# aditya-v-kallappa/FInCFlow

Hardware: AMD Instinct MI355X
Metric: inverse images/sec (+ fwd+logdet ms/img in `forward`), 3x3 conv @64x64x96 (higher is better)
Workload: dtype f32

## Files before the change

fincflow_amd/_lib.py:

```python
import ctypes
import os

HERE = os.path.dirname(os.path.abspath(__file__))
LIB_OVERRIDE = os.environ.get("FINCFLOW_LIB") or None
LIB_PATH = LIB_OVERRIDE or os.path.join(HERE, "libfinc_hip.so")

OK = 0
ALGO = {"auto": 0, "strict": 1, "mfma": 2}

SYMBOLS = [
    "finc_version", "finc_status_string", "finc_last_hip_error", "finc_canonicalize_weights_f32",
    "finc_check_invariant_f32", "finc_workspace_bytes", "finc_inverse_algo_for", "finc_forward_algo_for",
    "finc_inverse_f32", "finc_forward_f32", "finc_pack_inverse_weights_f32", "finc_pack_forward_weights_f32",
    "finc_inverse_packed_f32", "finc_forward_packed_f32", "finc_backward_f32", "finc_backward_workspace_bytes",
    "finc_inverse_workspace_bytes", "finc_pack_inverse_weights_affine_f32",
    "finc_canonicalize_weights_f64", "finc_inverse_f64", "finc_forward_f64",
    "finc_f64_workspace_bytes", "finc_inverse_f64_algo", "finc_forward_f64_algo",
    "finc_inverse_kernel_variant", "finc_debug_attr_table_insert", "finc_debug_inverse_table_row",
    "finc_mix_supported_f32", "finc_mix_f32", "finc_pack_forward_weights_affine_f32", "finc_debug_hlp_timeouts",
    "finc_build_flags", "finc_inverse_packed_premultiplied_f32", "finc_inverse_premultiplied_supported", "finc_clear_fault", "finc_debug_backward_variant", "finc_debug_set_forward_form",
    "finc_debug_row_chunks", "finc_debug_inverse_remainder_images",
    "finc_inverse_affine_supported", "finc_fault_pending", "finc_runtime_switches",
    "finc_debug_clock_probe_begin", "finc_debug_clock_probe_end",
    "finc_mix_backward_workspace_bytes", "finc_mix_backward_f32",
    "finc_coupling_supported_f32", "finc_coupling_workspace_bytes", "finc_coupling_f32", "finc_coupling_backward_f32",
    "finc_bias_relu_f32",
    "finc_actnorm_workspace_bytes", "finc_actnorm_f32", "finc_actnorm_backward_f32", "finc_actnorm_init_f32",
    "finc_adjoint_weights_f32", "finc_lead_product_f32", "finc_negate_f32", "finc_inverse_backward_workspace_bytes",
    "finc_inverse_backward_f32",
    "finc_coupling_reverse_backward_f32", "finc_actnorm_reverse_backward_f32",
    "finc_coupling_reverse_logdet_f32", "finc_coupling_reverse_logdet_backward_f32",
]

ABI_VERSION = 104
ACTNORM_ABI_VERSION = 105
INVERSE_BACKWARD_ABI_VERSION = 107
REVERSE_BACKWARD_ABI_VERSION = 108
SAMPLE_LOGDET_ABI_VERSION = 109

_lib = None


class FincError(RuntimeError):
    pass


def lib():
    global _lib
    if _lib is not None:
        return _lib
    if not os.path.exists(LIB_PATH):
        raise FincError(
            f"{LIB_PATH} not found: build it with `python -c 'import __graft_entry__ as g; g.build()'` "
            "(or `make -C fincflow_amd/csrc`).  fincflow_amd has no CPU / PyTorch fallback.")
    L = ctypes.CDLL(LIB_PATH)
    vp, i, u, sz = ctypes.c_void_p, ctypes.c_int, ctypes.c_uint, ctypes.c_size_t
    try:
        L.finc_version.restype = i
        have = int(L.finc_version())
    except AttributeError:
        raise FincError(f"{LIB_PATH} does not export finc_version: not a build of libfinc_hip.so") from None
    if have < ABI_VERSION:
        raise FincError(f"{LIB_PATH} reports finc_version() = {have}, this package needs at least {ABI_VERSION}: rebuild it "
                        "(`make -C fincflow_amd/csrc`)" + (" or unset FINCFLOW_LIB" if LIB_OVERRIDE else ""))
    if have < ACTNORM_ABI_VERSION:
        raise FincError(f"{LIB_PATH} reports finc_version() = {have}, the ActNorm entry points (finc_actnorm_f32, "
                        f"finc_actnorm_backward_f32, finc_actnorm_init_f32) came with {ACTNORM_ABI_VERSION}: rebuild it "
                        "(`make -C fincflow_amd/csrc`)" + (" or unset FINCFLOW_LIB" if LIB_OVERRIDE else ""))
    if have < INVERSE_BACKWARD_ABI_VERSION:
        raise FincError(f"{LIB_PATH} reports finc_version() = {have}, the backward through the inverse (finc_adjoint_weights_f32, "
                        f"finc_inverse_backward_f32) came with {INVERSE_BACKWARD_ABI_VERSION}: rebuild it "
                        "(`make -C fincflow_amd/csrc`)" + (" or unset FINCFLOW_LIB" if LIB_OVERRIDE else ""))
    if have < REVERSE_BACKWARD_ABI_VERSION:
        raise FincError(f"{LIB_PATH} reports finc_version() = {have}, the backwards of the reverse direction "
                        f"(finc_coupling_reverse_backward_f32, finc_actnorm_reverse_backward_f32) came with "
                        f"{REVERSE_BACKWARD_ABI_VERSION}: rebuild it "
                        "(`make -C fincflow_amd/csrc`)" + (" or unset FINCFLOW_LIB" if LIB_OVERRIDE else ""))
    if have < SAMPLE_LOGDET_ABI_VERSION:
        raise FincError(f"{LIB_PATH} reports finc_version() = {have}, the coupling's reverse with its log-det "
                        f"(finc_coupling_reverse_logdet_f32, finc_coupling_reverse_logdet_backward_f32) came with "
                        f"{SAMPLE_LOGDET_ABI_VERSION}: rebuild it "
                        "(`make -C fincflow_amd/csrc`)" + (" or unset FINCFLOW_LIB" if LIB_OVERRIDE else ""))
    L.finc_build_flags.restype = u
    L.finc_clear_fault.restype = i
    L.finc_status_string.restype = ctypes.c_char_p
    L.finc_status_string.argtypes = [i]
    L.finc_last_hip_error.restype = ctypes.c_char_p
    L.finc_canonicalize_weights_f32.argtypes = [vp, vp, i, i, i, i, u, vp]
    L.finc_check_invariant_f32.argtypes = [vp, i, i, i, i, vp]
    L.finc_workspace_bytes.restype = sz
    L.finc_workspace_bytes.argtypes = [i, i, i, i]
    L.finc_inverse_algo_for.argtypes = [i, i, i, i, i]
    L.finc_forward_algo_for.argtypes = [i, i, i, i, i]
    run = [vp, vp, vp, i, i, i, i, i, i, i, u, i, vp, sz, vp]
    L.finc_inverse_f32.argtypes = run
    L.finc_forward_f32.argtypes = run
    L.finc_pack_inverse_weights_f32.argtypes = [vp, vp, i, i, i, i, vp]
    L.finc_pack_inverse_weights_affine_f32.argtypes = [vp, vp, vp, vp, i, i, i, i, vp]
    L.finc_pack_forward_weights_f32.argtypes = [vp, vp, i, i, i, i, vp]
    L.finc_pack_forward_weights_affine_f32.argtypes = [vp, vp, vp, vp, i, i, i, i, vp]
    runp = [vp, vp, vp, i, i, i, i, i, i, i, u, vp]
    L.finc_inverse_packed_f32.argtypes = runp
    L.finc_inverse_packed_premultiplied_f32.argtypes = runp
    L.finc_inverse_premultiplied_supported.argtypes = [i, i, i, i, i, i, i]
    L.finc_inverse_affine_supported.argtypes = [i, i, i, i, i, i, i]
    L.finc_fault_pending.restype = i
    L.finc_runtime_switches.argtypes = [ctypes.c_char_p, sz]
    L.finc_debug_clock_probe_begin.argtypes = [i, i]
    L.finc_debug_clock_probe_end.argtypes = [ctypes.POINTER(ctypes.c_double)]
    L.finc_forward_packed_f32.argtypes = runp
    L.finc_backward_workspace_bytes.restype = sz
    L.finc_inverse_workspace_bytes.restype = sz
    L.finc_inverse_workspace_bytes.argtypes = [i, i, i, i, i, i, i]
    L.finc_backward_workspace_bytes.argtypes = [i, i, i, i, i, i, i]
# ... 10 lines not shown
    L.finc_debug_attr_table_insert.argtypes = [i, sz]
    L.finc_debug_inverse_table_row.argtypes = [i, ctypes.POINTER(ctypes.c_int)]
    L.finc_debug_hlp_timeouts.argtypes = [ctypes.POINTER(ctypes.c_uint)]
    L.finc_debug_backward_variant.argtypes = [i, i, i, i, i, i, i, ctypes.POINTER(ctypes.c_int)]
    L.finc_debug_inverse_remainder_images.argtypes = [i, i, i, i, i, i, i]
    L.finc_debug_row_chunks.argtypes = [ctypes.c_longlong, ctypes.c_longlong, i, i, i, i]
    L.finc_debug_set_forward_form.argtypes = [i]
    L.finc_mix_supported_f32.argtypes = [i]
    L.finc_mix_f32.argtypes = [vp, vp, vp, vp, i, i, i, vp]
    L.finc_mix_backward_workspace_bytes.restype = sz
    L.finc_mix_backward_workspace_bytes.argtypes = [i, i, i]
    L.finc_mix_backward_f32.argtypes = [vp, vp, vp, vp, vp, vp, i, i, i, vp, sz, vp]
    L.finc_coupling_supported_f32.argtypes = [i]
    L.finc_coupling_workspace_bytes.restype = sz
    L.finc_coupling_workspace_bytes.argtypes = [i, i, i]
    L.finc_coupling_f32.argtypes = [vp, vp, vp, vp, vp, vp, i, i, i, i, vp, sz, vp]
    L.finc_coupling_backward_f32.argtypes = [vp, vp, vp, vp, vp, vp, vp, vp, vp, vp, i, i, i, vp, sz, vp]
    L.finc_bias_relu_f32.argtypes = [vp, vp, vp, i, i, i, vp]
    L.finc_actnorm_workspace_bytes.restype = sz
    L.finc_actnorm_workspace_bytes.argtypes = [i, i, i]
    L.finc_actnorm_f32.argtypes = [vp, vp, vp, vp, vp, i, i, i, i, vp]
    L.finc_actnorm_backward_f32.argtypes = [vp, vp, vp, vp, vp, vp, vp, i, i, i, vp, sz, vp]
    L.finc_actnorm_init_f32.argtypes = [vp, vp, vp, i, i, i, vp, sz, vp]
    L.finc_adjoint_weights_f32.argtypes = [vp, vp, vp, i, i, i, i, vp]
    L.finc_lead_product_f32.argtypes = [vp, vp, i, i, i, i, vp]
    L.finc_negate_f32.argtypes = [vp, sz, vp]
    L.finc_inverse_backward_workspace_bytes.restype = sz
    L.finc_inverse_backward_workspace_bytes.argtypes = [i, i, i, i, i, i, i]
    L.finc_inverse_backward_f32.argtypes = [vp, vp, vp, vp, vp, i, i, i, i, i, i, i, u, vp, sz, vp]
    L.finc_coupling_reverse_backward_f32.argtypes = [vp, vp, vp, vp, vp, vp, vp, vp, vp, i, i, i, vp, sz, vp]
    L.finc_actnorm_reverse_backward_f32.argtypes = [vp, vp, vp, vp, vp, vp, i, i, i, vp, sz, vp]
    L.finc_coupling_reverse_logdet_f32.argtypes = [vp, vp, vp, vp, vp, vp, i, i, i, vp, sz, vp]
    L.finc_coupling_reverse_logdet_backward_f32.argtypes = [vp, vp, vp, vp, vp, vp, vp, vp, vp, vp, i, i, i, vp, sz, vp]
    for name in SYMBOLS:
        getattr(L, name)
    _lib = L
    if LIB_OVERRIDE:
        import sys
        print(f"fincflow_amd: FINCFLOW_LIB override -> {LIB_PATH} (finc_build_flags = {int(L.finc_build_flags()):#x})", file=sys.stderr)
    return L


def library_info():
    return {"path": os.path.relpath(LIB_PATH, os.path.dirname(HERE)) if not LIB_OVERRIDE else LIB_PATH,
            "env_override": bool(LIB_OVERRIDE), "build_flags": int(lib().finc_build_flags()), "version": int(lib().finc_version())}


def inverse_variant(B, G, Cq, H, W, KH, KW):
    info = (ctypes.c_int * 8)()
    st = lib().finc_inverse_kernel_variant(B, G, Cq, H, W, KH, KW, info)
    if st == 3:
        return None
    check(st, "finc_inverse_kernel_variant")
    keys = ("cqp", "nw", "npw", "sec", "lds_bytes", "workgroups", "row", "rows")
    return dict(zip(keys, list(info)))


def inverse_remainder_images(B, G, Cq, H, W, KH, KW):
    return int(lib().finc_debug_inverse_remainder_images(B, G, Cq, H, W, KH, KW))


def backward_variant(B, G, Cq, H, W, KH, KW):
    info = (ctypes.c_int * 3)()
    check(lib().finc_debug_backward_variant(B, G, Cq, H, W, KH, KW, info), "finc_debug_backward_variant")
    form = "scalar" if info[1] == 0 else ("strip", "strip16", "winograd", "msplit", "winograd4", "winograd25", "winograd4m", "stream")[info[2]]
    return {"gradw": ("direct", "dword", "staged", "tiled", "winograd", "winograd_tiled")[info[0]], "gradx_waves": info[1],
            "conv_form": form}


def set_forward_form(form):
    check(lib().finc_debug_set_forward_form(int(form)), "finc_debug_set_forward_form")


def build_flags():
    return int(lib().finc_build_flags())


def runtime_switches():
    buf = ctypes.create_string_buffer(1024)
    n = lib().finc_runtime_switches(buf, len(buf))
    return [t for t in buf.value.decode().split(",") if t] if n else []


def clock_probe_begin(period_us=250, max_ms=3000):
    check(lib().finc_debug_clock_probe_begin(int(period_us), int(max_ms)), "finc_debug_clock_probe_begin")


def clock_probe_end():
    st = (ctypes.c_double * 6)()
    check(lib().finc_debug_clock_probe_end(st), "finc_debug_clock_probe_end")
    return {"mean_mhz": st[0], "min_mhz": st[1], "max_mhz": st[2], "samples": int(st[3]), "seconds": st[4], "median_mhz": st[5]}

# ... 40 lines not shown
```

fincflow_amd/csrc/finc_abi.hip:

```cpp
#include "finc_common.h"

#include <stdlib.h>
#include <string.h>

#include <atomic>
#include <mutex>
#include <utility>
#include <vector>

namespace {

thread_local char g_hip_error[256] = "no error";

std::mutex g_table_mutex;
std::vector<std::pair<int, const void *>> g_attr_done;
constexpr int MAX_DEVICES = 64;
int *g_invariant_flag[MAX_DEVICES];
volatile unsigned *g_fault_host[MAX_DEVICES];
unsigned *g_fault_dev[MAX_DEVICES];
std::vector<std::pair<int, size_t>> g_debug_tokens;

std::atomic<bool> g_fault_armed_any{false};
std::vector<const char *> g_env_seen;

// ... 118 lines not shown
                if (e) { (void)hipHostFree(h); return e; }
                g_fault_dev[dev] = d;
                g_fault_host[dev] = h;
                g_fault_armed_any.store(true, std::memory_order_release);
            }
            w = g_fault_host[dev];
        }
    }
    if (w && *w != 0) {
        strncpy(g_hip_error, "a helper-wave wait of an earlier launch on this device gave up: its output is not valid (finc_clear_fault() resets)",
                sizeof(g_hip_error) - 1);
        return FINC_ERR_LAUNCH;
    }
    return FINC_OK;
}

template <typename T>
static int canonicalize(const T *w_stored, T *w_canon, int G, int Cq, int KH, int KW, unsigned orient, finc_stream_t stream)
{
    if (!w_stored || !w_canon) return FINC_ERR_NULL_POINTER;
    if (int e = check_shape(1, G, Cq, 1, 1, KH, KW)) return e;
    if (w_stored == w_canon) return FINC_ERR_BAD_DIMS;
    const int total = G * Cq * Cq * KH * KW;
    int blocks = (total + 255) / 256;
    if (blocks > 1024) blocks = 1024;
    hipLaunchKernelGGL(canonicalize_kernel<T>, dim3(blocks), dim3(256), 0, (hipStream_t)stream, w_stored, w_canon, G,
                       Cq, KH, KW, orient);
    FINC_CHECK_LAUNCH();
    return FINC_OK;
}

extern "C" {

int finc_version(void) { return 109; }

unsigned finc_build_flags(void)
{
    return FINC_BUILD_FLAGS | finc_build_flags_mfma() | finc_build_flags_split() | finc_build_flags_chain() | finc_build_flags_f64() | finc_build_flags_conv() | finc_build_flags_gradw() | finc_build_flags_wino4m() |
           finc_build_flags_mix() | finc_build_flags_generic() | finc_build_flags_wino() | finc_build_flags_big() | finc_build_flags_probe() | finc_build_flags_wino5() | finc_build_flags_stream();
}

int finc_fault_pending(void)
{
    int dev = 0;
    if (hipGetDevice(&dev) != hipSuccess || dev < 0 || dev >= MAX_DEVICES) return 0;
    volatile unsigned *w = g_fault_host[dev];
    return (w && *w != 0) ? 1 : 0;
}

int finc_runtime_switches(char *h_buf, size_t n)
{
    std::lock_guard<std::mutex> lk(g_table_mutex);
    size_t used = 0;
    int count = 0;
    auto put = [&](const char *t) {
        const size_t l = strlen(t);
        if (h_buf && used + l + 2 < n) {
            if (used) h_buf[used++] = ',';
            memcpy(h_buf + used, t, l);
            used += l;
        }
        ++count;
    };
    for (const char *name : g_env_seen) put(name);
    if (finc_wino_form_override() != 0) put("forward_form_override");
    if (h_buf && n) h_buf[used < n ? used : n - 1] = 0;
    return count;
// ... 412 lines not shown
    if (!finc_coupling_supported_f32(C)) return FINC_ERR_UNSUPPORTED;
    if (workspace_short(workspace, workspace_bytes, finc_coupling_workspace_bytes(B, C, HW))) return FINC_ERR_WORKSPACE;
    if (int e = finc_fault_gate(false)) return e;
    return finc_coupling_reverse_logdet_launch(x, raw, a, b, y, logdet, B, C, HW, (float *)workspace, (hipStream_t)stream);
}

int finc_coupling_reverse_logdet_backward_f32(const float *grad_y, const float *grad_logdet, const float *y, const float *raw,
                                              const float *a, const float *b, float *grad_x, float *grad_raw, float *grad_a,
                                              float *grad_b, int B, int C, int HW, void *workspace, size_t workspace_bytes,
                                              finc_stream_t stream)
{
    if (!grad_y || !y || !raw || !a || !b || (!grad_x && !grad_raw && !grad_a && !grad_b)) return FINC_ERR_NULL_POINTER;
    if (int e = pixel_dims(B, C, HW, true)) return e;
    if (grad_x && (grad_x == grad_y || grad_x == y || grad_x == raw)) return FINC_ERR_BAD_DIMS;
    if (grad_raw && (grad_raw == grad_y || grad_raw == y || grad_raw == raw || grad_raw == grad_x)) return FINC_ERR_BAD_DIMS;
    if (misaligned(grad_y, grad_logdet, y, raw, a, b, grad_x, grad_raw, grad_a, grad_b)) return FINC_ERR_ALIGNMENT;
    if (!finc_coupling_supported_f32(C)) return FINC_ERR_UNSUPPORTED;
    if ((grad_a || grad_b) && workspace_short(workspace, workspace_bytes, finc_coupling_workspace_bytes(B, C, HW)))
        return FINC_ERR_WORKSPACE;
    if (int e = finc_fault_gate(false)) return e;
    return finc_coupling_reverse_backward_launch(grad_y, grad_logdet, y, raw, a, b, grad_x, grad_raw, grad_a, grad_b, B, C, HW,
                                                 (float *)workspace, (hipStream_t)stream);
}

int finc_bias_relu_f32(const float *in, const float *bias, float *out, int B, int C, int HW, finc_stream_t stream)
{
    if (!in || !bias || !out) return FINC_ERR_NULL_POINTER;
    if (int e = pixel_dims(B, C, HW, false)) return e;
    if (misaligned(in, bias, out)) return FINC_ERR_ALIGNMENT;
    if (int e = finc_fault_gate(false)) return e;
    return finc_bias_relu_launch(in, bias, out, B, C, HW, (hipStream_t)stream);
}

size_t finc_actnorm_workspace_bytes(int B, int C, int HW)
{
    return pixel_counts_bad(B, C, HW, false) ? 256 : padded_ws_bytes(finc_actnorm_workspace_floats(B, C, HW) * sizeof(float));
}

int finc_actnorm_f32(const float *x, const float *log_scale, const float *translation, float *y, float *logdet, int B, int C, int HW,
                     int direction, finc_stream_t stream)
{
    if (!x || !log_scale || !translation || !y) return FINC_ERR_NULL_POINTER;
    if (int e = pixel_dims(B, C, HW, true)) return e;
    if (direction != 1 && direction != -1) return FINC_ERR_BAD_DIMS;
    if (misaligned(x, log_scale, translation, y, logdet)) return FINC_ERR_ALIGNMENT;
    if (int e = finc_fault_gate(false)) return e;
    return finc_actnorm_launch(x, log_scale, translation, y, direction > 0 ? logdet : nullptr, B, C, HW, direction, (hipStream_t)stream);
}

int finc_actnorm_backward_f32(const float *grad_y, const float *grad_logdet, const float *y, const float *log_scale, float *grad_x,
                              float *grad_log_scale, float *grad_translation, int B, int C, int HW, void *workspace,
                              size_t workspace_bytes, finc_stream_t stream)
{
    if (!grad_y || !y || !log_scale || (!grad_x && !grad_log_scale && !grad_translation)) return FINC_ERR_NULL_POINTER;
    if (int e = pixel_dims(B, C, HW, true)) return e;
    if (grad_x && grad_x == y) return FINC_ERR_BAD_DIMS;
    if (misaligned(grad_y, grad_logdet, y, log_scale, grad_x, grad_log_scale, grad_translation)) return FINC_ERR_ALIGNMENT;
    if ((grad_log_scale || grad_translation) && workspace_short(workspace, workspace_bytes, finc_actnorm_workspace_bytes(B, C, HW)))
        return FINC_ERR_WORKSPACE;
    if (int e = finc_fault_gate(false)) return e;
    return finc_actnorm_backward_launch(grad_y, grad_logdet, y, log_scale, grad_x, grad_log_scale, grad_translation, B, C, HW,
                                        (float *)workspace, (hipStream_t)stream);
}

int finc_actnorm_reverse_backward_f32(const float *grad_y, const float *x, const float *log_scale, float *grad_x, float *grad_log_scale,
                                      float *grad_translation, int B, int C, int HW, void *workspace, size_t workspace_bytes,
// ... 197 lines not shown
```

fincflow_amd/csrc/finc_common.h:

```cpp
#pragma once
#include <hip/hip_runtime.h>
#include <stddef.h>
#include <stdint.h>

#include "../../include/finc.h"
#include "finc_experiment.h"

#define FINC_FLIP_W 1u
#define FINC_FLIP_H 2u

__host__ __device__ inline unsigned finc_group_orient(unsigned orient, int g) { return (orient >> (2 * g)) & 3u; }

__device__ inline int finc_pix(int H, int W, unsigned o, int h, int w)
{
    int hh = (o & FINC_FLIP_H) ? H - 1 - h : h;
    int ww = (o & FINC_FLIP_W) ? W - 1 - w : w;
    return hh * W + ww;
}

void finc_set_hip_error(hipError_t e);

#define FINC_HIP_TRY(expr)                     \
    do {                                       \
        hipError_t _e = (expr);                \
// ... 153 lines not shown
    dim3 rgrid;
    size_t bytes = 0;
};
FincGradwPlan finc_gradw_plan(const FincShape &s, int align);
int finc_gradw_launch(const float *gz, const float *x, float *gw, void *workspace, const FincShape &s, const FincGradwPlan &p,
                      hipStream_t st);
int finc_gradw_variant(const FincShape &s);
size_t finc_gradw_workspace_bytes(const FincShape &s);
size_t finc_gradw_workspace_bound(int G, int Cq, int KH, int KW, long long units);

bool finc_f64_supported(const FincShape &s);
size_t finc_f64_packed_bytes(int G, int Cq, int KH, int KW);
int finc_f64_launch(const double *in, const double *wc, double *out, void *packed, const FincShape &s, bool forward, hipStream_t st);
unsigned finc_build_flags_f64();

bool finc_mix_supported(int C);
int finc_mix_launch(const float *in, const float *mat, const float *bias, float *out, int B, int C, int HW, hipStream_t st,
                    bool transposed = false);
size_t finc_mix_gradw_workspace_bytes(int B, int C, int HW);
int finc_mix_gradw_launch(const float *grad_out, const float *in, float *gm, float *gb, void *workspace, int B, int C, int HW,
                          int align, hipStream_t st);

size_t finc_coupling_workspace_floats(int B, int C, int HW);
int finc_coupling_launch(const float *x, const float *raw, const float *a, const float *b, float *y, float *logdet, int B, int C, int HW,
                         int direction, float *ws, hipStream_t st);
int finc_coupling_backward_launch(const float *gy, const float *gld, const float *x, const float *raw, const float *a, const float *b,
                                  float *gx, float *graw, float *ga, float *gb, int B, int C, int HW, float *ws, hipStream_t st);
int finc_coupling_reverse_logdet_launch(const float *x, const float *raw, const float *a, const float *b, float *y, float *logdet, int B,
                                        int C, int HW, float *ws, hipStream_t st);
int finc_coupling_reverse_backward_launch(const float *gy, const float *gld, const float *y, const float *raw, const float *a,
                                          const float *b, float *gx, float *graw, float *ga, float *gb, int B, int C, int HW, float *ws,
                                          hipStream_t st);
int finc_bias_relu_launch(const float *in, const float *bias, float *out, int B, int C, int HW, hipStream_t st);
size_t finc_actnorm_workspace_floats(int B, int C, int HW);
int finc_actnorm_launch(const float *x, const float *ls, const float *tr, float *y, float *logdet, int B, int C, int HW, int direction,
                        hipStream_t st);
int finc_actnorm_backward_launch(const float *gy, const float *gld, const float *y, const float *ls, float *gx, float *gls, float *gt,
                                 int B, int C, int HW, float *ws, hipStream_t st);
int finc_actnorm_reverse_backward_launch(const float *gy, const float *x, const float *ls, float *gx, float *gls, float *gt, int B, int C,
                                         int HW, float *ws, hipStream_t st);
int finc_actnorm_init_launch(const float *x, float *ls, float *tr, int B, int C, int HW, float *ws, hipStream_t st);
int finc_adjoint_weights_launch(const float *wc, float *w_adj, float *lead_t, int G, int Cq, int KH, int KW, hipStream_t st);
int finc_lead_launch(float *v, const float *lead_t, int B, int G, int Cq, int HW, hipStream_t st);
int finc_negate_launch(float *p, size_t n, hipStream_t st);
```

fincflow_amd/csrc/finc_mix.hip:

```cpp
#include "finc_common.h"

namespace {

typedef float v4f __attribute__((ext_vector_type(4)));
typedef float v2f __attribute__((ext_vector_type(2)));

constexpr unsigned MIX_INVALID = 0x80000000u;

template <int PX>
struct PixVec;
template <>
struct PixVec<1> {
    static __device__ inline void load(float (&d)[1], __amdgpu_buffer_rsrc_t r, unsigned voff, int soff)
    {
        d[0] = __builtin_bit_cast(float, __builtin_amdgcn_raw_buffer_load_b32(r, voff, soff, 0));
    }
    static __device__ inline void store(const float (&d)[1], __amdgpu_buffer_rsrc_t r, unsigned voff, int soff)
    {
        __builtin_amdgcn_raw_buffer_store_b32(__builtin_bit_cast(unsigned, d[0]), r, voff, soff, 0);
    }
};
template <>
struct PixVec<2> {
    typedef unsigned v2u __attribute__((ext_vector_type(2)));
// ... 160 lines not shown
    if (!m) return FINC_ERR_UNSUPPORTED;
    if ((size_t)C * HW * 4 >= ((size_t)1 << 31)) return FINC_ERR_BAD_DIMS;
    const size_t lds = (size_t)((C + 15) / 16) * (C / 4 + 1) * 64 * sizeof(float);
    const uintptr_t ptrs = (uintptr_t)in | (uintptr_t)out;
    const long long chunks1 = (long long)B * ((HW + 15) / 16);
    const int big = chunks1 >= 4LL * 256 * 16 ? 1 : 0;
    int pxi = (HW % 4 == 0 && (ptrs & 15u) == 0 && HW >= 64) ? 2 : (HW % 2 == 0 && (ptrs & 7u) == 0 && HW >= 32) ? 1 : 0;
    int wb = big;
    while (pxi > 0 && !m->fn[pxi][wb]) {
        if (m->fn[pxi][wb ^ 1]) { wb ^= 1; break; }
        --pxi;
    }
    if (!m->fn[pxi][wb]) wb ^= 1;
    const mix_fn fn = m->fn[pxi][wb];
    if (!fn) return FINC_ERR_UNSUPPORTED;
    const int px = 1 << pxi;
    const int wgw = lds > 80 * 1024 ? 16 : wb == 0 ? 4 : pxi == 2 ? 8 : 16;
    const int cpi = (HW + 16 * px - 1) / (16 * px);
    const long long total = (long long)B * cpi;
    if (total >= (1LL << 31)) return FINC_ERR_BAD_DIMS;
    if (int e = finc_ensure_dynamic_lds((const void *)fn, lds)) return e;
    const int waves_cu = pxi == 2 ? 8 : 16;
    int wgs_per_cu = (int)((160 * 1024) / lds);
    if (wgs_per_cu > waves_cu / wgw) wgs_per_cu = waves_cu / wgw;
    if (wgs_per_cu < 1) wgs_per_cu = 1;
    long long wgs = (total + wgw - 1) / wgw;
    if (wgs > 256LL * wgs_per_cu) wgs = 256LL * wgs_per_cu;
    hipLaunchKernelGGL(fn, dim3((unsigned)wgs), dim3(64 * wgw), lds, st, in, mat, bias, out, C, HW, cpi, (int)total, transposed ? 1 : 0);
    FINC_CHECK_LAUNCH();
    return FINC_OK;
}

#include "finc_coupling.h"
#include "finc_actnorm.h"
#include "finc_adjoint.h"

unsigned finc_build_flags_mix() { return FINC_BUILD_FLAGS; }
```

fincflow_amd/glow.py:

```python
import math

import numpy as np
import torch
import torch.nn as nn
import torch.nn.functional as F

from . import ops
from .layers import FastFlowUnit, FlowLayer, FlowSequential, _hip_tensor, _records_graph


class Squeeze(FlowLayer):
    def forward(self, input, context=None):
        b, c, h, w = input.shape
        x = input.reshape(b, c, h // 2, 2, w // 2, 2).permute(0, 1, 3, 5, 2, 4)
        return x.reshape(b, c * 4, h // 2, w // 2), self.logdet(input, context)

    def reverse(self, input, context=None):
        b, c, h, w = input.shape
        x = input.reshape(b, c // 4, 2, 2, h, w).permute(0, 1, 4, 2, 5, 3)
        return x.reshape(b, c // 4, h * 2, w * 2)

    def reverse_with_logdet(self, input, context=None):
        return self.reverse(input, context), input.new_zeros(len(input))

# ... 227 lines not shown

    def _hip_reverse_grad(self, x, context=None):
        return ops.reverse_grad_enabled() and self._hip_train(x, context)

    def _raw_train(self, x, context):
        n = self.net
        return F.conv2d(n[:4](self._net_input(x, context)), n[4].weight, None, padding=1)

    def _scale_shift(self):
        last = self.net[4]
        a = torch.exp(last.logs * last.logscale_factor)
        return a, last.bias * a

    def _scale_shift_cached(self):
        last = self.net[4]
        key = ops.version_key(last.logs, last.bias) + (last.logs.device,)
        if getattr(self, "_ab_key", None) == key:
            return self._ab
        with torch.no_grad():
            a, b = self._scale_shift()
            ab = (a.contiguous(), b.contiguous())
        if not torch.cuda.is_current_stream_capturing():
            self._ab, self._ab_key = ab, key
        return ab

    def _net_input(self, x, context):
        assert (context is not None) == self.uses_context
        x1 = x[:, :self.half_channels]
        return x1 if context is None else torch.cat([x1, context], dim=1)

    def _raw_inference(self, x, context):
        n = self.net
        with torch.no_grad():
            h = F.conv2d(self._net_input(x, context), n[0].weight, None, padding=1).contiguous()
            ops.finc_bias_relu(h, n[0].bias.detach(), out=h)
            h = F.conv2d(h, n[2].weight, None).contiguous()
            ops.finc_bias_relu(h, n[2].bias.detach(), out=h)
            return F.conv2d(h, n[4].weight, None, padding=1).contiguous()

    def _params(self, x, context):
        assert (context is not None) == self.uses_context
        x1, x2 = x[:, :self.half_channels], x[:, self.half_channels:]
        h = self.net(x1 if context is None else torch.cat([x1, context], dim=1))
        log_s = 2.0 * torch.tanh(h[:, ::2] / 2.0)
        return x1, x2, log_s, h[:, 1::2]

    def forward(self, input, context=None):
        if self._hip(input, context):
            x = input.contiguous()
            a, b = self._scale_shift_cached()
            return ops.finc_coupling(x, self._raw_inference(x, context), a, b, 1, True)
        if self._hip_train(input, context):
            a, b = self._scale_shift()
            return ops.coupling_forward(input, self._raw_train(input, context), a, b)
        x1, x2, log_s, t = self._params(input, context)
        return torch.cat([x1, x2 * torch.exp(log_s) + t], dim=1), log_s.flatten(start_dim=1).sum(-1)

    def reverse(self, input, context=None):
        if self._hip(input, context):
            x = input.contiguous()
            a, b = self._scale_shift_cached()
            return ops.finc_coupling(x, self._raw_inference(x, context), a, b, -1, False)[0]
        if self._hip_reverse_grad(input, context):
            a, b = self._scale_shift()
            return ops.coupling_reverse(input, self._raw_train(input, context), a, b)
        x1, x2, log_s, t = self._params(input, context)
        return torch.cat([x1, (x2 - t) * torch.exp(-log_s)], dim=1)

# ... 142 lines not shown
```

fincflow_amd/ops.py:

```python
import contextlib
import threading

import torch
from torch.optim.optimizer import register_optimizer_step_post_hook

from . import _lib

ORDER_BITS = {"TL": 0, "TR": 1, "BL": 2, "BR": 3}
ORIENT_FASTFLOW = 0xE4

_workspaces = {}
_reverse_grad = threading.local()


@contextlib.contextmanager
def reverse_grad():
    depth = getattr(_reverse_grad, "depth", 0)
    _reverse_grad.depth = depth + 1
    try:
        yield
    finally:
        _reverse_grad.depth = depth


# ... 396 lines not shown

class _FincCouplingReverseLogdetFunction(torch.autograd.Function):

    @staticmethod
    def forward(ctx, x, raw, a, b):
        x, raw, a, b = x.contiguous(), raw.contiguous(), a.contiguous(), b.contiguous()
        y, logdet = finc_coupling_reverse_logdet(x, raw, a, b)
        ctx.save_for_backward(y, raw, a, b)
        return y, logdet

    @staticmethod
    @torch.autograd.function.once_differentiable
    def backward(ctx, grad_y, grad_logdet):
        y, raw, a, b = ctx.saved_tensors
        need = ctx.needs_input_grad
        return finc_coupling_reverse_logdet_backward(*_incoming_grads(y, grad_y, grad_logdet), y, raw, a, b,
                                                     need_gx=need[0], need_graw=need[1], need_ga=need[2], need_gb=need[3])


def coupling_reverse_logdet(x, raw, a, b):
    return _FincCouplingReverseLogdetFunction.apply(x, raw, a, b)


def finc_bias_relu(x, bias, out=None):
    _require_device(x, "input")
    _require_device(bias, "bias")
    if x.dim() != 4 or bias.numel() != x.shape[1] or bias.device != x.device:
        raise ValueError("expected activations [B,C,H,W] and one bias entry per channel on the same device")
    out = _out_like(x, out)
    if x.numel() == 0:
        return out
    B, C, H, W = x.shape
    _call("finc_bias_relu_f32", x.device, x.data_ptr(), bias.data_ptr(), out.data_ptr(), B, C, H * W, _stream_ptr(x))
    return out


def actnorm_supported():
    _lib.lib()
    return True


def _actnorm_args(x, log_scale, translation, what="input"):
    _require_device(x, what)
    _require_device(log_scale, "log_scale")
    if x.dim() != 4:
        raise ValueError(f"expected {what} [B,C,H,W]")
    _per_channel(x, "log_scale", log_scale)
    if translation is not None:
        _require_device(translation, "translation")
        _per_channel(x, "translation", translation)


def finc_actnorm(x, log_scale, translation, direction=1, want_logdet=False, out=None):
    _actnorm_args(x, log_scale, translation)
    if direction not in (1, -1):
        raise ValueError("direction must be +1 (forward) or -1 (reverse)")
    out = _out_like(x, out)
    B, C, H, W = x.shape
    want_logdet = bool(want_logdet) and direction == 1
    if x.numel() == 0:
        return out, (torch.zeros(B, dtype=torch.float32, device=x.device) if want_logdet else None)
    logdet = torch.empty(B, dtype=torch.float32, device=x.device) if want_logdet else None
    _call("finc_actnorm_f32", x.device, x.data_ptr(), log_scale.data_ptr(), translation.data_ptr(), out.data_ptr(), _ptr(logdet), B, C,
          H * W, direction, _stream_ptr(x))
    return out, logdet

# ... 370 lines not shown
```

include/finc.h:

```cpp
#ifndef FINC_H
#define FINC_H

#include <stddef.h>

#ifdef __cplusplus
extern "C" {
#endif

typedef void *finc_stream_t;

enum finc_status {
    FINC_OK = 0,
    FINC_ERR_NULL_POINTER = 1,
    FINC_ERR_BAD_DIMS = 2,
    FINC_ERR_UNSUPPORTED = 3,
    FINC_ERR_WORKSPACE = 4,
    FINC_ERR_LAUNCH = 5,
    FINC_ERR_INVARIANT = 6,
    FINC_ERR_ALIGNMENT = 7
};

enum finc_algo {
    FINC_ALGO_AUTO = 0,
    FINC_ALGO_STRICT = 1,
// ... 68 lines not shown
size_t finc_f64_workspace_bytes(int G, int Cq, int KH, int KW);
int finc_inverse_f64_algo(const double *z, const double *w_canon, double *x, int B, int G, int Cq, int H, int W, int KH, int KW,
                          unsigned orient, int algo, void *workspace, size_t workspace_bytes, finc_stream_t stream);
int finc_forward_f64_algo(const double *x, const double *w_canon, double *z, int B, int G, int Cq, int H, int W, int KH, int KW,
                          unsigned orient, int algo, void *workspace, size_t workspace_bytes, finc_stream_t stream);

int finc_mix_supported_f32(int C);
int finc_mix_f32(const float *in, const float *mat, const float *bias, float *out, int B, int C, int HW,
                 finc_stream_t stream);

size_t finc_mix_backward_workspace_bytes(int B, int C, int HW);
int finc_mix_backward_f32(const float *grad_out, const float *in, const float *mat, float *grad_in, float *grad_mat,
                          float *grad_bias, int B, int C, int HW, void *workspace, size_t workspace_bytes,
                          finc_stream_t stream);

int finc_coupling_supported_f32(int C);
size_t finc_coupling_workspace_bytes(int B, int C, int HW);
int finc_coupling_f32(const float *x, const float *raw, const float *a, const float *b, float *y, float *logdet, int B, int C,
                      int HW, int direction, void *workspace, size_t workspace_bytes, finc_stream_t stream);
int finc_coupling_backward_f32(const float *grad_y, const float *grad_logdet, const float *x, const float *raw, const float *a,
                               const float *b, float *grad_x, float *grad_raw, float *grad_a, float *grad_b, int B, int C, int HW,
                               void *workspace, size_t workspace_bytes, finc_stream_t stream);
int finc_coupling_reverse_backward_f32(const float *grad_y, const float *y, const float *raw, const float *a, const float *b,
                                       float *grad_x, float *grad_raw, float *grad_a, float *grad_b, int B, int C, int HW,
                                       void *workspace, size_t workspace_bytes, finc_stream_t stream);
int finc_coupling_reverse_logdet_f32(const float *x, const float *raw, const float *a, const float *b, float *y, float *logdet,
                                     int B, int C, int HW, void *workspace, size_t workspace_bytes, finc_stream_t stream);
int finc_coupling_reverse_logdet_backward_f32(const float *grad_y, const float *grad_logdet, const float *y, const float *raw,
                                              const float *a, const float *b, float *grad_x, float *grad_raw, float *grad_a,
                                              float *grad_b, int B, int C, int HW, void *workspace, size_t workspace_bytes,
                                              finc_stream_t stream);
int finc_bias_relu_f32(const float *in, const float *bias, float *out, int B, int C, int HW, finc_stream_t stream);

size_t finc_actnorm_workspace_bytes(int B, int C, int HW);
int finc_actnorm_f32(const float *x, const float *log_scale, const float *translation, float *y, float *logdet, int B, int C, int HW,
                     int direction, finc_stream_t stream);
int finc_actnorm_backward_f32(const float *grad_y, const float *grad_logdet, const float *y, const float *log_scale, float *grad_x,
                              float *grad_log_scale, float *grad_translation, int B, int C, int HW, void *workspace,
                              size_t workspace_bytes, finc_stream_t stream);
int finc_actnorm_reverse_backward_f32(const float *grad_y, const float *x, const float *log_scale, float *grad_x, float *grad_log_scale,
                                      float *grad_translation, int B, int C, int HW, void *workspace, size_t workspace_bytes,
                                      finc_stream_t stream);
int finc_actnorm_init_f32(const float *x, float *log_scale, float *translation, int B, int C, int HW, void *workspace,
                          size_t workspace_bytes, finc_stream_t stream);

int finc_inverse_kernel_variant(int B, int G, int Cq, int H, int W, int KH, int KW, int *info);
int finc_debug_backward_variant(int B, int G, int Cq, int H, int W, int KH, int KW, int *info);
int finc_debug_set_forward_form(int form);
int finc_debug_inverse_remainder_images(int B, int G, int Cq, int H, int W, int KH, int KW);
int finc_debug_row_chunks(long long units, long long slots, int H, int min_rows, int extra, int second_tenant);
int finc_debug_inverse_table_row(int row, int *info);
int finc_debug_attr_table_insert(int device, size_t kernel_token);
int finc_debug_hlp_timeouts(unsigned *h_count);
int finc_clear_fault(void);
int finc_fault_pending(void);
int finc_runtime_switches(char *h_buf, size_t n);
int finc_debug_clock_probe_begin(int period_us, int max_ms);
int finc_debug_clock_probe_end(double *h_stats);

#ifdef __cplusplus
}
#endif
#endif
```

Baseline: 645,700.

## Add fused MFMA 3x3 conv + bias + ReLU kernel for coupling net's first layer

Adds a HIP kernel that stages padded input images in LDS and computes the coupling net's first 3x3 convolution with fp32 MFMA, fusing bias and ReLU into the store. It reads the half-channel slice directly through a batch stride, so the input slicing copy, the separate conv2d, and the bias_relu pass are all avoided. The inference path uses it when there is no context and the shape fits. It adds a planner for images per workgroup and tile variants, plus many template instantiations. It only covers small Cin and Cout divisible by 64.

```diff
diff --git a/fincflow_amd/_lib.py b/fincflow_amd/_lib.py
--- a/fincflow_amd/_lib.py
+++ b/fincflow_amd/_lib.py
@@ -30,6 +30,7 @@
     "finc_inverse_backward_f32",
     "finc_coupling_reverse_backward_f32", "finc_actnorm_reverse_backward_f32",
     "finc_coupling_reverse_logdet_f32", "finc_coupling_reverse_logdet_backward_f32",
+    "finc_netconv_supported", "finc_conv3x3_bias_relu_f32", "finc_debug_netconv_plan",
 ]
 
 ABI_VERSION = 104
@@ -37,6 +38,7 @@
 INVERSE_BACKWARD_ABI_VERSION = 107
 REVERSE_BACKWARD_ABI_VERSION = 108
 SAMPLE_LOGDET_ABI_VERSION = 109
+NETCONV_ABI_VERSION = 110
 
 _lib = None
 
@@ -80,6 +82,10 @@
         raise FincError(f"{LIB_PATH} reports finc_version() = {have}, the coupling's reverse with its log-det "
                         f"(finc_coupling_reverse_logdet_f32, finc_coupling_reverse_logdet_backward_f32) came with "
                         f"{SAMPLE_LOGDET_ABI_VERSION}: rebuild it "
+                        "(`make -C fincflow_amd/csrc`)" + (" or unset FINCFLOW_LIB" if LIB_OVERRIDE else ""))
+    if have < NETCONV_ABI_VERSION:
+        raise FincError(f"{LIB_PATH} reports finc_version() = {have}, the coupling net's fused first convolution "
+                        f"(finc_netconv_supported, finc_conv3x3_bias_relu_f32) came with {NETCONV_ABI_VERSION}: rebuild it "
                         "(`make -C fincflow_amd/csrc`)" + (" or unset FINCFLOW_LIB" if LIB_OVERRIDE else ""))
     L.finc_build_flags.restype = u
     L.finc_clear_fault.restype = i
@@ -156,6 +162,9 @@
     L.finc_actnorm_reverse_backward_f32.argtypes = [vp, vp, vp, vp, vp, vp, i, i, i, vp, sz, vp]
     L.finc_coupling_reverse_logdet_f32.argtypes = [vp, vp, vp, vp, vp, vp, i, i, i, vp, sz, vp]
     L.finc_coupling_reverse_logdet_backward_f32.argtypes = [vp, vp, vp, vp, vp, vp, vp, vp, vp, vp, i, i, i, vp, sz, vp]
+    L.finc_netconv_supported.argtypes = [i, i, i, i]
+    L.finc_conv3x3_bias_relu_f32.argtypes = [vp, ctypes.c_longlong, vp, vp, vp, i, i, i, i, i, vp]
+    L.finc_debug_netconv_plan.argtypes = [i, i, i, i, i, i, ctypes.POINTER(ctypes.c_int)]
     for name in SYMBOLS:
         getattr(L, name)
     _lib = L
@@ -182,6 +191,15 @@
 
 def inverse_remainder_images(B, G, Cq, H, W, KH, KW):
     return int(lib().finc_debug_inverse_remainder_images(B, G, Cq, H, W, KH, KW))
+
+
+def netconv_plan(B, Cin, Cout, H, W, out_aligned16=True):
+    info = (ctypes.c_int * 8)()
+    st = lib().finc_debug_netconv_plan(B, Cin, Cout, H, W, 1 if out_aligned16 else 0, info)
+    if st == 3:
+        return None
+    check(st, "finc_debug_netconv_plan")
+    return dict(zip(("images", "groups", "slices", "workgroups", "lds_bytes", "nkb", "px", "mt"), list(info)))
 
 
 def backward_variant(B, G, Cq, H, W, KH, KW):
diff --git a/fincflow_amd/csrc/finc_abi.hip b/fincflow_amd/csrc/finc_abi.hip
--- a/fincflow_amd/csrc/finc_abi.hip
+++ b/fincflow_amd/csrc/finc_abi.hip
@@ -174,7 +174,7 @@
 
 extern "C" {
 
-int finc_version(void) { return 109; }
+int finc_version(void) { return 110; }
 
 unsigned finc_build_flags(void)
 {
@@ -653,6 +653,29 @@
     return finc_bias_relu_launch(in, bias, out, B, C, HW, (hipStream_t)stream);
 }
 
+int finc_conv3x3_bias_relu_f32(const float *x, long long x_batch_stride, const float *weight, const float *bias, float *out, int B,
+                               int Cin, int Cout, int H, int W, finc_stream_t stream)
+{
+    if (!x || !weight || !bias || !out) return FINC_ERR_NULL_POINTER;
+    if (B <= 0 || Cin <= 0 || Cout <= 0 || H <= 0 || W <= 0) return FINC_ERR_BAD_DIMS;
+    if (misaligned(x, weight, bias, out)) return FINC_ERR_ALIGNMENT;
+    if (!finc_netconv_supported(Cin, Cout, H, W)) return FINC_ERR_UNSUPPORTED;
+    if (x_batch_stride < (long long)Cin * H * W || x_batch_stride >= (1LL << 40) || pixel_total_bad(B, Cout, H * W)) return FINC_ERR_BAD_DIMS;
+    if (int e = finc_fault_gate(false)) return e;
+    return finc_netconv_launch(x, x_batch_stride, weight, bias, out, B, Cin, Cout, H, W, (hipStream_t)stream);
+}
+
+int finc_debug_netconv_plan(int B, int Cin, int Cout, int H, int W, int out_aligned16, int *info)
+{
+    if (!info) return FINC_ERR_NULL_POINTER;
+    if (B <= 0 || Cin <= 0 || Cout <= 0 || H <= 0 || W <= 0) return FINC_ERR_BAD_DIMS;
+    FincNetconvPlan pl;
+    if (int e = finc_netconv_plan(B, Cin, Cout, H, W, out_aligned16 != 0, &pl)) return e;
+    info[0] = pl.images; info[1] = pl.groups; info[2] = pl.slices; info[3] = (int)pl.grid; info[4] = (int)pl.lds_bytes;
+    info[5] = pl.nkb; info[6] = pl.px; info[7] = pl.mt;
+    return FINC_OK;
+}
+
 size_t finc_actnorm_workspace_bytes(int B, int C, int HW)
 {
     return pixel_counts_bad(B, C, HW, false) ? 256 : padded_ws_bytes(finc_actnorm_workspace_floats(B, C, HW) * sizeof(float));
diff --git a/fincflow_amd/csrc/finc_common.h b/fincflow_amd/csrc/finc_common.h
--- a/fincflow_amd/csrc/finc_common.h
+++ b/fincflow_amd/csrc/finc_common.h
@@ -209,6 +209,14 @@
                                           const float *b, float *gx, float *graw, float *ga, float *gb, int B, int C, int HW, float *ws,
                                           hipStream_t st);
 int finc_bias_relu_launch(const float *in, const float *bias, float *out, int B, int C, int HW, hipStream_t st);
+struct FincNetconvPlan {
+    int images, groups, slices, nkb, px, mt;
+    unsigned grid;
+    size_t lds_bytes;
+};
+int finc_netconv_plan(int B, int Cin, int Cout, int H, int W, bool out_aligned16, FincNetconvPlan *plan);
+int finc_netconv_launch(const float *x, long long x_batch_stride, const float *weight, const float *bias, float *out, int B, int Cin,
+                        int Cout, int H, int W, hipStream_t st);
 size_t finc_actnorm_workspace_floats(int B, int C, int HW);
 int finc_actnorm_launch(const float *x, const float *ls, const float *tr, float *y, float *logdet, int B, int C, int HW, int direction,
                         hipStream_t st);
diff --git a/fincflow_amd/csrc/finc_mix.hip b/fincflow_amd/csrc/finc_mix.hip
--- a/fincflow_amd/csrc/finc_mix.hip
+++ b/fincflow_amd/csrc/finc_mix.hip
@@ -216,6 +216,7 @@
 }
 
 #include "finc_coupling.h"
+#include "finc_netconv.h"
 #include "finc_actnorm.h"
 #include "finc_adjoint.h"
 
diff --git a/fincflow_amd/csrc/finc_netconv.h b/fincflow_amd/csrc/finc_netconv.h
--- /dev/null
+++ b/fincflow_amd/csrc/finc_netconv.h
@@ -0,0 +1,228 @@
+#ifndef FINC_NETCONV_H
+#define FINC_NETCONV_H
+
+#include <stdlib.h>
+#include <string.h>
+
+namespace {
+
+typedef float ncv_v4f __attribute__((ext_vector_type(4)));
+
+constexpr int NCV_THREADS = 256;
+constexpr int NCV_SLICE = 64;
+constexpr int NCV_MAX_K = 256;
+constexpr long long NCV_MAX_STAGED = 64 * 1024;
+
+__device__ inline int ncv_div(int n, float rd) { return (int)(((float)n + 0.5f) * rd); }
+
+template <int NKB, int PX, int MT>
+__global__ __launch_bounds__(NCV_THREADS) void finc_netconv_kernel(const float *__restrict__ x, long long x_batch_stride,
+                                                                   const float *__restrict__ wgt, const float *__restrict__ bias,
+                                                                   float *__restrict__ out, int B, int Cin, int Cout, int H, int W,
+                                                                   int images)
+{
+    constexpr int NK = 4 * NKB;
+    extern __shared__ __attribute__((aligned(16))) float ncv_lds[];
+    const int HW = H * W, W2 = W + 2, PS = (H + 2) * W2, IS = Cin * PS, K = 9 * Cin;
+    const int slices = Cout / NCV_SLICE;
+    const int grp = (int)blockIdx.x / slices, slice = (int)blockIdx.x - grp * slices;
+    const int i0 = grp * images, ni = B - i0 < images ? B - i0 : images, npix = ni * HW;
+    float *const simg = ncv_lds;
+    unsigned *const spix = reinterpret_cast<unsigned *>(ncv_lds + ((images * IS + 3) & ~3));
+    const int lane = threadIdx.x & 63, q = lane >> 4, p = lane & 15;
+    const int wave = __builtin_amdgcn_readfirstlane((int)(threadIdx.x >> 6));
+    const int c0 = slice * NCV_SLICE + (MT == 2 ? 32 * (wave & 1) : 16 * wave);
+    float a[MT][NK];
+    unsigned tap[NK / 2];
+#pragma unroll
+    for (int mt = 0; mt < MT; ++mt) {
+        const float *wrow = wgt + (size_t)(c0 + 16 * mt + p) * K;
+#pragma unroll
+        for (int m = 0; m < NKB - 1; ++m) {
+            float v[4];
+            __builtin_memcpy(v, wrow + 16 * m + 4 * q, 16);
+#pragma unroll
+            for (int jj = 0; jj < 4; ++jj) a[mt][4 * m + jj] = v[jj];
+        }
+#pragma unroll
+        for (int jj = 0; jj < 4; ++jj) {
+            const int k = 16 * (NKB - 1) + 4 * q + jj;
+            const float v = wrow[k < K ? k : K - 1];
+            a[mt][4 * (NKB - 1) + jj] = k < K ? v : 0.f;
+        }
+    }
+    float bv[MT][4];
+#pragma unroll
+    for (int mt = 0; mt < MT; ++mt)
+#pragma unroll
+        for (int r = 0; r < 4; ++r) bv[mt][r] = bias[c0 + 16 * mt + 4 * q + r];
+    {
+        constexpr int SU = 8;
+        const float rIS = 1.f / (float)IS, rPS = 1.f / (float)PS, rW2 = 1.f / (float)W2, rHW = 1.f / (float)HW, rW = 1.f / (float)W;
+        const float *const x0 = x + (size_t)i0 * (size_t)x_batch_stride;
+        const int nst = ni * IS;
+        for (int e0 = (int)threadIdx.x; e0 < nst; e0 += NCV_THREADS * SU) {
+            float v[SU];
+            bool inside[SU];
+#pragma unroll
+            for (int u = 0; u < SU; ++u) {
+                const int e = e0 + u * NCV_THREADS < nst ? e0 + u * NCV_THREADS : 0;
+                const int il = ncv_div(e, rIS), r = e - il * IS, ic = ncv_div(r, rPS), r2 = r - ic * PS, hh = ncv_div(r2, rW2), ww = r2 - hh * W2;
+                inside[u] = hh >= 1 && hh <= H && ww >= 1 && ww <= W;
+                const size_t src = (size_t)il * (size_t)x_batch_stride + (size_t)ic * HW + (size_t)((hh - 1) * W + (ww - 1));
+                v[u] = x0[inside[u] ? src : 0];
+            }
+#pragma unroll
+            for (int u = 0; u < SU; ++u)
+                if (e0 + u * NCV_THREADS < nst) simg[e0 + u * NCV_THREADS] = inside[u] ? v[u] : 0.f;
+        }
+        for (int e = (int)threadIdx.x; e < npix; e += NCV_THREADS) {
+            const int il = ncv_div(e, rHW), r = e - il * HW, h = ncv_div(r, rW), w = r - h * W;
+            spix[e] = (unsigned)(il * IS + h * W2 + w) * 4u;
+        }
+    }
+#pragma unroll
+    for (int j = 0; j < NK; ++j) {
+        const int k = 16 * (j / 4) + 4 * q + (j & 3);
+        const int ic = k / 9, t = k - 9 * ic, dy = t / 3, dx = t - 3 * dy;
+        const unsigned off = k < K ? (unsigned)(ic * PS + dy * W2 + dx) * 4u : 0u;
+        if (j & 1) tap[j / 2] |= off << 16;
+        else tap[j / 2] = off;
+    }
+    __syncthreads();
+    const char *const sbytes = reinterpret_cast<const char *>(simg);
+    auto tap_of = [&](int j) { return (j & 1) ? tap[j / 2] >> 16 : tap[j / 2] & 0xffffu; };
+    constexpr int PER = 16 * PX;
+    const float rHW = 1.f / (float)HW;
+    for (int t0 = (MT == 2 ? (wave >> 1) * PER : 0); t0 < npix; t0 += MT * PER) {
+        const int pix = t0 + PX * p;
+        const bool ok = pix < npix;
+        unsigned po[PX];
+        if constexpr (PX == 4) {
+            const uint4 v = *reinterpret_cast<const uint4 *>(spix + (ok ? pix : 0));
+            po[0] = v.x; po[1] = v.y; po[2] = v.z; po[3] = v.w;
+        } else {
+            po[0] = spix[ok ? pix : 0];
+        }
+        ncv_v4f acc[MT][PX];
+        float bc[PX], bn[PX];
+#pragma unroll
+        for (int e = 0; e < PX; ++e) {
+#pragma unroll
+            for (int mt = 0; mt < MT; ++mt) acc[mt][e] = (ncv_v4f){0.f, 0.f, 0.f, 0.f};
+            bc[e] = *reinterpret_cast<const float *>(sbytes + (tap_of(0) + po[e]));
+        }
+#pragma unroll
+        for (int j = 0; j < NK; ++j) {
+            if (j + 1 < NK) {
+                const unsigned to = tap_of(j + 1);
+#pragma unroll
+                for (int e = 0; e < PX; ++e) bn[e] = *reinterpret_cast<const float *>(sbytes + (to + po[e]));
+            }
+            __builtin_amdgcn_sched_barrier(0);
+            if (j >= NK - 4) {
+                const bool real = 16 * (NKB - 1) + 4 * q + (j & 3) < K;
+#pragma unroll
+                for (int e = 0; e < PX; ++e) bc[e] = real ? bc[e] : 0.f;
+            }
+#pragma unroll
+            for (int mt = 0; mt < MT; ++mt)
+#pragma unroll
+                for (int e = 0; e < PX; ++e) acc[mt][e] = __builtin_amdgcn_mfma_f32_16x16x4f32(a[mt][j], bc[e], acc[mt][e], 0, 0, 0);
+            __builtin_amdgcn_sched_barrier(0);
+#pragma unroll
+            for (int e = 0; e < PX; ++e) bc[e] = bn[e];
+        }
+        if (!ok) continue;
+        const int il = ncv_div(pix, rHW), hw = pix - il * HW;
+#pragma unroll
+        for (int mt = 0; mt < MT; ++mt) {
+            float *orow = out + ((size_t)(i0 + il) * Cout + (size_t)(c0 + 16 * mt + 4 * q)) * HW + hw;
+#pragma unroll
+            for (int r = 0; r < 4; ++r) {
+                float d[PX];
+#pragma unroll
+                for (int e = 0; e < PX; ++e) {
+                    const float s = (r == 0 ? acc[mt][e].x : r == 1 ? acc[mt][e].y : r == 2 ? acc[mt][e].z : acc[mt][e].w) + bv[mt][r];
+                    d[e] = s != s ? s : fmaxf(s, 0.f);
+                }
+                cpl_store<PX>(orow + (size_t)r * HW, d);
+            }
+        }
+    }
+}
+
+typedef void (*ncv_fn)(const float *, long long, const float *, const float *, float *, int, int, int, int, int, int);
+
+constexpr int NCV_MT2_NKB = 7;
+#define NCV_ROW7(PX, MT, N0)                                                                                                        \
+    finc_netconv_kernel<N0 + 1, PX, MT>, finc_netconv_kernel<N0 + 2, PX, MT>, finc_netconv_kernel<N0 + 3, PX, MT>,                     \
+        finc_netconv_kernel<N0 + 4, PX, MT>, finc_netconv_kernel<N0 + 5, PX, MT>, finc_netconv_kernel<N0 + 6, PX, MT>,                 \
+        finc_netconv_kernel<N0 + 7, PX, MT>
+#define NCV_ROW16(PX) {NCV_ROW7(PX, 1, 0), NCV_ROW7(PX, 1, 7), finc_netconv_kernel<15, PX, 1>, finc_netconv_kernel<16, PX, 1>}
+const ncv_fn g_ncv[3][16] = {NCV_ROW16(1), NCV_ROW16(4), {NCV_ROW7(4, 2, 0)}};
+#undef NCV_ROW16
+#undef NCV_ROW7
+
+inline long long ncv_lds_bytes(int Cin, int H, int W, int images)
+{
+    const long long staged = (long long)images * Cin * (H + 2) * (W + 2);
+    return (((staged + 3) & ~3LL) + (long long)images * H * W) * 4;
+}
+
+}
+
+int finc_netconv_supported(int Cin, int Cout, int H, int W)
+{
+    if (Cin < 1 || Cout < 1 || H < 1 || W < 1) return 0;
+    if (Cout % NCV_SLICE != 0 || 9LL * Cin > NCV_MAX_K) return 0;
+    return (long long)Cin * ((long long)H + 2) * ((long long)W + 2) * 4 <= NCV_MAX_STAGED ? 1 : 0;
+}
+
+constexpr int NCV_PIXELS = 256, NCV_WGS = 512, NCV_LDS_CAP = 64 * 1024;
+
+int finc_netconv_plan(int B, int Cin, int Cout, int H, int W, bool out_aligned16, FincNetconvPlan *plan)
+{
+    if (B < 1 || !finc_netconv_supported(Cin, Cout, H, W)) return FINC_ERR_UNSUPPORTED;
+    const int HW = H * W;
+    FincNetconvPlan pl;
+    pl.px = (HW % 4 == 0 && out_aligned16) ? 4 : 1;
+    pl.nkb = ((9 * Cin + 3) / 4 + 3) / 4;
+    pl.slices = Cout / NCV_SLICE;
+    long long ni = (NCV_PIXELS + HW - 1) / HW;
+    if (ni > B) ni = B;
+    while (ni > 1 && ncv_lds_bytes(Cin, H, W, (int)ni) > NCV_LDS_CAP) --ni;
+    while (ni > 1 && ((B + ni - 1) / ni) * pl.slices < NCV_WGS && ((ni + 1) / 2) * HW >= 64) ni = (ni + 1) / 2;
+    if (const char *s = finc_env("FINC_NETCONV_IMAGES")) {
+        const long long v = atoll(s);
+        if (v >= 1 && v <= B && (v == 1 || ncv_lds_bytes(Cin, H, W, (int)v) <= NCV_LDS_CAP)) ni = v;
+    }
+    pl.images = (int)ni;
+    pl.groups = (int)((B + ni - 1) / ni);
+    pl.mt = (pl.px == 4 && pl.nkb <= NCV_MT2_NKB && ni * HW >= 2 * 64) ? 2 : 1;
+    if (const char *s = finc_env("FINC_NETCONV_MT")) {
+        const int v = atoi(s);
+        if (v == 1 || (v == 2 && pl.px == 4 && pl.nkb <= NCV_MT2_NKB)) pl.mt = v;
+    }
+    const long long grid = (long long)pl.groups * pl.slices;
+    if (grid >= (1LL << 31)) return FINC_ERR_BAD_DIMS;
+    pl.grid = (unsigned)grid;
+    pl.lds_bytes = (size_t)ncv_lds_bytes(Cin, H, W, pl.images);
+    *plan = pl;
+    return FINC_OK;
+}
+
+int finc_netconv_launch(const float *x, long long x_batch_stride, const float *weight, const float *bias, float *out, int B, int Cin,
+                        int Cout, int H, int W, hipStream_t st)
+{
+    FincNetconvPlan pl;
+    if (int e = finc_netconv_plan(B, Cin, Cout, H, W, ((uintptr_t)out & 15u) == 0, &pl)) return e;
+    const ncv_fn fn = g_ncv[pl.px == 4 ? pl.mt : 0][pl.nkb - 1];
+    if (int e = finc_ensure_dynamic_lds((const void *)fn, pl.lds_bytes)) return e;
+    hipLaunchKernelGGL(fn, dim3(pl.grid), dim3(NCV_THREADS), pl.lds_bytes, st, x, x_batch_stride, weight, bias, out, B, Cin, Cout, H, W,
+                       pl.images);
+    FINC_CHECK_LAUNCH();
+    return FINC_OK;
+}
+
+#endif
diff --git a/fincflow_amd/glow.py b/fincflow_amd/glow.py
--- a/fincflow_amd/glow.py
+++ b/fincflow_amd/glow.py
@@ -283,8 +283,11 @@
     def _raw_inference(self, x, context):
         n = self.net
         with torch.no_grad():
-            h = F.conv2d(self._net_input(x, context), n[0].weight, None, padding=1).contiguous()
-            ops.finc_bias_relu(h, n[0].bias.detach(), out=h)
+            if context is None and ops.netconv_supported(self.half_channels, self.width, x.shape[2], x.shape[3]):
+                h = ops.finc_conv3x3_bias_relu(x, self.half_channels, n[0].weight.detach(), n[0].bias.detach())
+            else:
+                h = F.conv2d(self._net_input(x, context), n[0].weight, None, padding=1).contiguous()
+                ops.finc_bias_relu(h, n[0].bias.detach(), out=h)
             h = F.conv2d(h, n[2].weight, None).contiguous()
             ops.finc_bias_relu(h, n[2].bias.detach(), out=h)
             return F.conv2d(h, n[4].weight, None, padding=1).contiguous()
diff --git a/fincflow_amd/ops.py b/fincflow_amd/ops.py
--- a/fincflow_amd/ops.py
+++ b/fincflow_amd/ops.py
@@ -452,6 +452,34 @@
         return out
     B, C, H, W = x.shape
     _call("finc_bias_relu_f32", x.device, x.data_ptr(), bias.data_ptr(), out.data_ptr(), B, C, H * W, _stream_ptr(x))
+    return out
+
+
+def netconv_supported(cin, cout, H, W):
+    return bool(_lib.lib().finc_netconv_supported(int(cin), int(cout), int(H), int(W)))
+
+
+def finc_conv3x3_bias_relu(x, cin, weight, bias):
+    _require_device(x, "input")
+    _require_device(weight, "weight")
+    _require_device(bias, "bias")
+    cin = int(cin)
+    if x.dim() != 4 or not 1 <= cin <= x.shape[1]:
+        raise ValueError("expected activations [B,C,H,W] with at least `cin` channels")
+    if weight.dim() != 4 or tuple(weight.shape[1:]) != (cin, 3, 3) or bias.numel() != weight.shape[0]:
+        raise ValueError("expected a weight [cout, cin, 3, 3] and one bias entry per output channel")
+    if weight.device != x.device or bias.device != x.device:
+        raise ValueError("weight and bias must be on the activations' device")
+    B, C, H, W = x.shape
+    cout = weight.shape[0]
+    out = torch.empty((B, cout, H, W), dtype=torch.float32, device=x.device)
+    if out.numel() == 0:
+        return out
+    if not netconv_supported(cin, cout, H, W):
+        raise _lib.FincError(f"finc_conv3x3_bias_relu: no kernel for {cin} -> {cout} channels on {H}x{W} maps "
+                             "(ops.netconv_supported)")
+    _call("finc_conv3x3_bias_relu_f32", x.device, x.data_ptr(), C * H * W, weight.data_ptr(), bias.data_ptr(), out.data_ptr(),
+          B, cin, cout, H, W, _stream_ptr(x))
     return out
 
 
diff --git a/include/finc.h b/include/finc.h
--- a/include/finc.h
+++ b/include/finc.h
@@ -124,6 +124,10 @@
                                               finc_stream_t stream);
 int finc_bias_relu_f32(const float *in, const float *bias, float *out, int B, int C, int HW, finc_stream_t stream);
 
+int finc_netconv_supported(int Cin, int Cout, int H, int W);
+int finc_conv3x3_bias_relu_f32(const float *x, long long x_batch_stride, const float *weight, const float *bias, float *out, int B,
+                               int Cin, int Cout, int H, int W, finc_stream_t stream);
+
 size_t finc_actnorm_workspace_bytes(int B, int C, int HW);
 int finc_actnorm_f32(const float *x, const float *log_scale, const float *translation, float *y, float *logdet, int B, int C, int HW,
                      int direction, finc_stream_t stream);
@@ -141,6 +145,7 @@
 int finc_debug_set_forward_form(int form);
 int finc_debug_inverse_remainder_images(int B, int G, int Cq, int H, int W, int KH, int KW);
 int finc_debug_row_chunks(long long units, long long slots, int H, int min_rows, int extra, int second_tenant);
+int finc_debug_netconv_plan(int B, int Cin, int Cout, int H, int W, int out_aligned16, int *info);
 int finc_debug_inverse_table_row(int row, int *info);
 int finc_debug_attr_table_insert(int device, size_t kernel_token);
 int finc_debug_hlp_timeouts(unsigned *h_count);
```

New measurement: 645,700 (median of 2 runs). No clear change (-0.0%).
